# thawro/pytorch-human-pose

Measured on AMD Instinct MI355X. Metric: images/sec (fwd+decode) HigherHRNet-W32 512px, higher is better.
Workload: dtype bf16; 1 GPU; HigherHRNet-W32 inference bf16, batch 32 @ 512x512 per GPU (conv fwd on N(0,1) images + AE decode on constructed maps, 10 people/image, det_thr 0.05, tag_thr 0.5, adjust+refine); global_batch=32, parallelism=image-sharded replicas x1, no data-path collective

## Files before the change

### pytorch-human-pose_amd/csrc/engine.cpp

```cpp
#include "engine.h"

#include <cmath>
#include <cstdlib>
#include <cstring>

static thread_local std::string g_err;
LaunchProbe &hh_launch_probe()
{
    static thread_local LaunchProbe p;
    return p;
}
void hh_set_error(const std::string &msg) { g_err = msg; }
const char *hh_get_error() { return g_err.c_str(); }

PlanSwitches PlanSwitches::from_env()
{
    auto on = [](const char *name) { const char *v = getenv(name); return v && *v && strcmp(v, "0"); };
    auto is = [](const char *name, const char *val) { const char *v = getenv(name); return v && !strcmp(v, val); };
    PlanSwitches s;
    s.bb32_tile = is("HH_BB32", "tile");
    s.no_bb64 = on("HH_NO_BB64");
    s.no_bb_fp8 = on("HH_NO_BB_FP8");
    s.no_stem_fused = on("HH_NO_STEM_FUSED");
    s.no_junc_pair = on("HH_NO_JUNC_PAIR");
    s.full_join = on("HH_FULL_JOIN");
    s.no_fusion_merge = on("HH_NO_FUSION_MERGE");
    s.no_fused_upsum = on("HH_NO_FUSED_UPSUM");
    s.poison_ws = on("HH_POISON_WS");
    s.poison_lds = on("HH_POISON_LDS");
    s.no_head_fold = on("HH_NO_HEAD_FOLD");
    s.no_conv_db = on("HH_NO_CONV_DB");
    s.no_final_fuse = on("HH_NO_FINAL_FUSE");
    s.keep_waits = on("HH_KEEP_WAITS");
    s.event_system_fence = on("HH_EVENT_SYSTEM_FENCE");
    s.bb_tall = on("HH_NO_BB_TALL") ? 0 : is("HH_BB_TALL", "always") ? 2 : 1;
    if (const char *fc = getenv("HH_FAT_CUS")) { s.fat_cus = s.fat_cus64 = atoi(fc); if (const char *c2 = strchr(fc, ',')) s.fat_cus64 = atoi(c2 + 1); }
    if (const char *sk = getenv("HH_DEBUG_SKIP")) {
        static const struct { const char *name; unsigned bit; } cats[] = {{"s2big", SK_S2BIG}, {"s2", SK_S2}, {"upadd", SK_UPADD}, {"c1x1", SK_C1X1},
            {"c256", SK_C256}, {"c128", SK_C128}, {"junc", SK_JUNC}, {"bb32", SK_BB32}, {"bb64", SK_BB64}, {"stem", SK_STEM}, {"deconv", SK_DECONV},
            {"head", SK_HEAD}, {"trans0", SK_TRANS0}, {"upsum", SK_UPSUM}};
        std::string v = std::string(",") + sk + ",";
        for (const auto &c : cats)
            if (v.find(std::string(",") + c.name + ",") != std::string::npos) s.debug_skip |= c.bit;
    }
    s.fp8_trunk8 = is("HH_FP8_TRUNK", "e4m3");
    s.fp8_heads8 = is("HH_FP8_HEADS", "e4m3");
    return s;
}

static inline int round_up(int v, int m) { return (v + m - 1) / m * m; }

static inline bf16_raw f2bf(float f)
{
    uint32_t u;
    memcpy(&u, &f, 4);
    if ((u & 0x7fffffffu) > 0x7f800000u) return (bf16_raw)((u >> 16) | 0x40);
    u += 0x7fffu + ((u >> 16) & 1u);
    return (bf16_raw)(u >> 16);
}
static inline float bf2f(bf16_raw h)
{
    uint32_t u = (uint32_t)h << 16;
    float f;
    memcpy(&f, &u, 4);
    return f;
}

int hh_net::add_param(const std::string &name, std::vector<int64_t> shape, bool counter)
{
    ParamSlot p;
    p.name = name;
    p.shape = std::move(shape);
    p.counter = counter;
    param_index[name] = (int)params.size();
    params.push_back(std::move(p));
    return (int)params.size() - 1;
// ... 501 lines not shown
                for (int c8 = 0; c8 < C8; ++c8)
                    for (int ci_o = 0; ci_o < COUT_T; ++ci_o)
                        for (int j = 0; j < 8; ++j, ++o) {
                            const int co = cg * COUT_T + ci_o, ci = ch * KC + c8 * 8 + j;
                            if (co >= cout || ci >= cin) continue;
                            float v;
                            if (transposed) v = W[(((size_t)ci * cout + co) * 4 + ky) * 4 + kx];
                            else v = W[(((size_t)co * cin + ci) * ks + ky) * ks + kx];
                            packed[o] = f2bf(v * scale[co]);
                        }
            }
}

int hh_family_pick(int ks, int stride, int cin_pad, int coutp, int *KC, int *NT)
{
    if (ks == 3 && stride == 1) *KC = (cin_pad % 32 == 0) ? 32 : 16;
    else if (ks == 1) *KC = (cin_pad % 32 == 0) ? 32 : 16;
    else *KC = 16;
    *NT = (coutp % 64 == 0) ? 2 : 1;
    for (int i = 0; i < conv_num_configs(); ++i) {
        const ConvConfig &c = conv_config(i);
        if (c.KS == ks && c.S == stride && c.KC == *KC && c.NT == *NT && !c.DB) return 0;
    }
    return 1;
}

float hh_net::bn_fold(const std::string &bn, int co, const float *cb, float *shift) const
{
    const float g = param(bn + ".weight")[co], bta = param(bn + ".bias")[co];
    const float mu = param(bn + ".running_mean")[co], var = param(bn + ".running_var")[co];
    const float sc = g / std::sqrt(var + 1e-5f);
    *shift = cb ? bta + (*cb - mu) * sc : bta - mu * sc;
    return sc;
}

void hh_net::fold_layer(const ConvLayer &l, int coutp, std::vector<float> &scale, std::vector<float> &shift) const
{
    scale.assign(coutp, 0.f);
    shift.assign(coutp, 0.f);
    for (int co = 0; co < l.cout; ++co) {
        const float cb = l.bias.empty() ? 0.f : param(l.bias)[co];
        if (l.bn.empty()) { scale[co] = 1.f; shift[co] = cb; }
        else scale[co] = bn_fold(l.bn, co, &cb, &shift[co]);
    }
}

int hh_net::finalize()
{
    for (auto &p : params)
        if (!p.loaded && !p.counter) { hh_set_error("hh_finalize: parameter never loaded: " + p.name); return 1; }
    HH_CHECK_HIP(conv_init());
    HH_CHECK_HIP(bb_fused_init());
    HH_CHECK_HIP(stem_fused_init());
    HH_CHECK_HIP(bbpc_init());
    HH_CHECK_HIP(bb64_fused_init());
    HH_CHECK_HIP(junction_init());
    if (dtype == 2 && kind != 0) { hh_set_error("hh_finalize: the fp8 path covers HigherHRNet only"); return 1; }
    {
        int dev = 0;
        hipDeviceProp_t prop;
        HH_CHECK_HIP(hipGetDevice(&dev));
        HH_CHECK_HIP(hipGetDeviceProperties(&prop, dev));
        num_cus = prop.multiProcessorCount;
    }
    for (auto &l : layers) {
        if (l.stem) {
            const std::vector<float> &W = param(l.conv + ".weight");
            std::vector<bf16_raw> packed(64 * 32, 0);
            std::vector<float> shift(64);
            for (int co = 0; co < 64; ++co) {
                const float sc = bn_fold(l.bn, co, nullptr, &shift[co]);
                for (int t = 0; t < 27; ++t) {
                    const int kk = t / 16, hh = (t % 16) / 8, j = t % 8;
                    packed[((((co / 32) * 2 + kk) * 2 + hh) * 32 + co % 32) * 8 + j] = f2bf(W[(size_t)co * 27 + t] * sc);
                }
            }
            if (hh_upload(&l.d_w, packed.data(), packed.size() * 2) || hh_upload(&l.d_bias, shift.data(), 64 * 4)) return 1;
            continue;
        }
        if (dtype == 2 && !l.hi) continue;
        const int cin_pad0 = round_up(l.cin, 16), coutp = round_up(l.cout, 32);
        if (l.stem2) { l.KC = 64; l.NT = 2; }
        else if (hh_family_pick(l.ks, l.stride, cin_pad0, coutp, &l.KC, &l.NT)) {
            hh_set_error("no kernel family for conv " + l.conv);
            return 1;
        }
        l.db = !sw.no_conv_db && !l.stem2 && l.ks == 3 && l.stride == 1 && !l.transposed && l.mconv.empty() && l.cin >= 128 &&
               l.cin % 16 == 0 && coutp % 64 == 0;
        if (l.db) { l.KC = 16; l.NT = 2; }
        l.cin_pad = round_up(l.cin, l.KC);
        const int COUT_T = 32 * l.NT;
        l.ncg = coutp / COUT_T;
        if (!l.mconv.empty()) {
            std::vector<float> Wm((size_t)l.cout * l.cin * 9, 0.f), one(coutp, 1.f), shift(coutp, 0.f);
            int c0 = 0;
            for (size_t m = 0; m < l.mconv.size(); ++m) {
                if (l.mcin[m] % l.KC) { hh_set_error("merged fusion conv: input width not a multiple of the chunk size"); return 1; }
                const std::vector<float> &Wj = param(l.mconv[m] + ".weight");
                for (int co = 0; co < l.cout; ++co) {
                    float sh;
                    const float sc = bn_fold(l.mbn[m], co, nullptr, &sh);
                    shift[co] += sh;
                    for (int ci = 0; ci < l.mcin[m]; ++ci)
                        for (int t = 0; t < 9; ++t) Wm[((size_t)co * l.cin + c0 + ci) * 9 + t] = Wj[((size_t)co * l.mcin[m] + ci) * 9 + t] * sc;
                }
                c0 += l.mcin[m];
// ... 267 lines not shown
            }
            HH_CHECK_HIP(launch_avgpool(ti.ptr, ti.C, d_pool, B, (H >> ti.shift) * (W >> ti.shift), op.C, s));
            break;
        }
        case OP_LINEAR:
            HH_CHECK_HIP(launch_linear(d_pool, d_fc_w, d_fc_b, o1, B, 2048, num_classes, s));
            break;
        case OP_STEM: rc = enqueue_stem(op, images, B, H, W, s); break;
        case OP_UPADD: rc = dtype == 2 ? enqueue_fp8_upadd(op, B, H, W, s) : enqueue_upadd(op, B, H, W, s); break;
        case OP_UPSUM: rc = enqueue_upsum(op, B, H, W, s); break;
        case OP_JUNC: rc = enqueue_junc(op, B, H, W, s); break;
        case OP_BB: rc = dtype == 2 ? enqueue_fp8_bb(op, B, H, W, s) : enqueue_bb(op, B, H, W, o2, multi, s, &fin_done); break;
        case OP_QUANT: rc = enqueue_fp8_quant(op, B, H, W, s); break;
        case OP_CONV: rc = dtype == 2 && !op.hi ? enqueue_fp8_conv(op, B, H, W, o1, o2, s) : enqueue_conv(op, B, H, W, o1, o2, s); break;
        }
        if (rc) return 1;
    }
    if (multi)
        for (int l = 1; l < lc.open; ++l)
            if ((lc.dep(0, l) || sw.keep_waits) && lane_wait(0, l)) return 1;
    return 0;
}

int hh_net::prof_record(const Op &op, int cfg, const OpCost &c, unsigned long long **clk)
{
    if (prof_used == prof.size()) {
        ProfRecord r{};
        HH_CHECK_HIP(hipEventCreate(&r.e0));
        HH_CHECK_HIP(hipEventCreate(&r.e1));
        prof.push_back(r);
    }
    ProfRecord &r = prof[prof_used++];
    r.op = (int)(&op - ops.data());
    r.cfg = cfg;
    r.flops = c.flops;
    r.bytes = c.bytes;
    r.slot = clk && prof_used <= HH_PROF_SLOTS ? (int)prof_used - 1 : -1;
    if (r.slot >= 0 && prof_clk) *clk = d_clk + 4 * r.slot;
    hh_launch_probe() = LaunchProbe{r.e0, r.e1};
    return 0;
}

int hh_net::enqueue_stem(const Op &op, const float *images, int B, int H, int W, hipStream_t s)
{
    const ConvLayer &l = layers[op.layer];
    if (op.layer2 >= 0) {
        const ConvLayer &l2 = layers[op.layer2];
        StemFusedParams q{};
        q.images = images; q.w1 = l.d_w; q.b1 = l.d_bias; q.w2 = l2.d_w; q.b2 = l2.d_bias;
        q.out = tensors[op.out].ptr; q.out_cs = tensors[op.out].C;
        q.B = B; q.H = H; q.W = W;
        if (!stem_fused_supported(q)) { hh_set_error("hh_forward: the fused stem needs H, W multiples of 4 and images below 2 GB (HH_NO_STEM_FUSED=1)"); return 1; }
        if (prof_enabled && prof_record(op, HH_CFG_STEM_FUSED, op_cost(op, B, H, W), &q.clk)) return 1;
        HH_CHECK_HIP(stem_fused_launch(q, num_cus, s));
        return 0;
    }
    StemParams p{};
    p.images = images; p.w = l.d_w; p.bias = l.d_bias;
    p.out = tensors[op.out].ptr; p.out_cs = tensors[op.out].C;
    p.B = B; p.H = H; p.W = W;
    if (dtype == 2) {
        p.out_fp8 = (unsigned char *)tensors[op.out].ptr; p.out_inv_scale = 1.f / op.s_out;
        if (calibrating) p.absmax = d_amax + (&op - ops.data());
    }
    if (prof_enabled && prof_record(op, HH_CFG_STEM, op_cost(op, B, H, W), &p.clk)) return 1;
    HH_CHECK_HIP(stem_conv_launch(p, s));
    return 0;
}

int hh_net::enqueue_upadd(const Op &op, int B, int H, int W, hipStream_t s)
{
    UpAddParams p{};
    const TensorDesc &b = tensors[op.in], &o = tensors[op.out];
    p.base = b.ptr; p.base_cs = b.C; p.base_coff = 0;
    p.nup = op.nup;
    for (int j = 0; j < op.nup; ++j) {
        p.up[j] = tensors[op.up[j]].ptr; p.up_cs[j] = tensors[op.up[j]].C; p.up_shift[j] = op.up_shift[j];
    }
    p.out = o.ptr; p.out_cs = o.C; p.out_coff = 0;
    p.B = B; p.H = H >> b.shift; p.W = W >> b.shift; p.C = op.C; p.relu = op.relu;
    HH_CHECK_HIP(launch_upadd(p, s));
    return 0;
}

int hh_net::enqueue_upsum(const Op &op, int B, int H, int W, hipStream_t s)
{
    const TensorDesc &b0 = tensors[op.in], &o = tensors[op.out];
    FusionUpParams p{};
    p.x0 = b0.ptr; p.x0_cs = b0.C;
    p.nsrc = op.nup;
    for (int j = 0; j < op.nup; ++j) {
        const ConvLayer &l = layers[op.up_layer[j]];
        const TensorDesc &t = tensors[op.up[j]];
        if (t.shift != b0.shift + j + 1 || l.KC != 32 || l.NT != 1 || l.ncg != 1 || l.cin != (op.C << (j + 1))) {
            hh_set_error("plan: fusion output 0 does not fit fusion_up.hip (HH_NO_FUSED_UPSUM=1)");
            return 1;
        }
        p.src[j] = t.ptr; p.src_cs[j] = t.C; p.w[j] = l.d_w; p.bias[j] = l.d_bias;
    }
    p.out = o.ptr; p.out_cs = o.C;
    p.B = B; p.H = H >> b0.shift; p.W = W >> b0.shift;
    if (prof_enabled && prof_record(op, HH_CFG_FUSION_UP, op_cost(op, B, H, W), &p.clk)) return 1;
    HH_CHECK_HIP(fusion_up_launch(p, s));
    return 0;
}

int hh_net::enqueue_junc(const Op &op, int B, int H, int W, hipStream_t s)
// ... 20 lines not shown
int hh_net::enqueue_bb(const Op &op, int B, int H, int W, float *o2, bool multi, hipStream_t s, int *fin_done)
{
    const ConvLayer &l1 = layers[op.layer], &l2 = layers[op.layer2];
    const TensorDesc &ti = tensors[op.in], &to = tensors[op.out];
    BBParams p{};
    p.in = ti.ptr; p.in_cs = ti.C; p.out = to.ptr; p.out_cs = to.C;
    p.w1 = l1.d_w; p.w2 = l2.d_w; p.b1 = l1.d_bias; p.b2 = l2.d_bias;
    p.B = B; p.H = H >> ti.shift; p.W = W >> ti.shift;
    p.tall = sw.bb_tall;
    if (op.fin >= 0 && !sw.no_final_fuse && !sw.bb32_tile && !taps_enabled && o2 && !(sw.debug_skip & SK_HEAD)) {
        const ConvLayer &lf = layers[ops[op.fin].layer];
        p.fin_w = lf.d_wfin; p.fin_b = lf.d_bias; p.fin_out = o2; p.fin_K = lf.cout;
        if (lf.d_wfin && bbpc_final_supported(p)) *fin_done = op.fin;
        else { p.fin_w = nullptr; p.fin_b = nullptr; p.fin_out = nullptr; p.fin_K = 0; }
    }
    const int cfg = l1.cout == 64 ? HH_CFG_BB64_FUSED : HH_CFG_BB_FUSED;
    if (prof_enabled && prof_record(op, cfg, op_cost(op, B, H, W, p.fin_out != nullptr), &p.clk)) return 1;
    auto budget = [&](int want) { return !(multi && op.siblings) ? num_cus : want > 0 ? (want < num_cus ? want : num_cus) : (num_cus + 1) / 2; };
    const int fat = budget(sw.fat_cus), fat64 = budget(sw.fat_cus64);
    if (l1.cout == 64) HH_CHECK_HIP(bb64_fused_launch(p, fat64, s));
    else if (!sw.bb32_tile && bbpc_supported(p)) HH_CHECK_HIP(bbpc_launch(p, fat, s));
    else HH_CHECK_HIP(bb_fused_launch(p, num_cus, s));
    return 0;
}

int hh_net::enqueue_conv(const Op &op, int B, int H, int W, float *o1, float *o2, hipStream_t s)
{
    const ConvLayer &l = layers[op.layer];
    const TensorDesc &ti = tensors[op.in];
    ConvParams p{};
    hh_conv_geometry(p, l, op, B, H >> ti.shift, W >> ti.shift, o1, o2);
    p.in = dtype == 2 ? ti.ptr16 : ti.ptr; p.in_cs = ti.C; p.in_coff = op.in_coff;
    p.w = l.d_w; p.bias = l.d_bias;
    if (op.out >= 0) {
        const TensorDesc &to = tensors[op.out];
        p.out = dtype == 2 ? to.ptr16 : to.ptr; p.out_cs = to.C; p.out_coff = op.out_coff;
    }
    if (op.res >= 0) {
        const TensorDesc &tr = tensors[op.res];
        p.res = dtype == 2 ? tr.ptr16 : tr.ptr; p.res_cs = tr.C; p.res_coff = op.res_coff;
    }
    if (op.in2 >= 0) {
        const TensorDesc &t2 = tensors[op.in2];
        if (t2.C != ti.C || t2.shift != ti.shift || (op.in3 >= 0 && (tensors[op.in3].C != ti.C || tensors[op.in3].shift != ti.shift))) {
            hh_set_error("merged fusion conv: inputs differ in shape or pixel stride");
            return 1;
        }
        p.nch0 = l.mcin[0] / l.KC;
        p.nch1 = l.mcin[1] / l.KC;
        p.src_delta1 = t2.ptr - (ti.ptr + op.in_coff);
        if (op.in3 >= 0) p.src_delta2 = tensors[op.in3].ptr - (ti.ptr + op.in_coff);
    }
    p.cout_store = op.cout_store >= 0 ? op.cout_store : round_up(l.cout, 8);
    const int cfg = hh_pick_config(l.ks, l.stride, l.KC, l.NT, p.Wo, l.db);
    const ConvConfig &c = conv_config(cfg);
    p.tiles_x = (p.Wo + c.TW - 1) / c.TW;
    p.tiles_y = (p.Ho + c.th() - 1) / c.th();
    if (prof_enabled && prof_record(op, cfg, op_cost(op, B, H, W), &p.clk)) return 1;
    HH_CHECK_HIP(conv_launch(cfg, p, s));
    return 0;
}

int hh_net::forward(const float *images, int B, int H, int W, float *o1, float *o2, int use_graph, hipStream_t s)
{
    if (!finalized) { hh_set_error("hh_forward: call hh_finalize first"); return 1; }
    if (dtype == 2 && !calibrated) { hh_set_error("hh_forward: fp8 handle without activation scales, call hh_calibrate first"); return 1; }
    if (B > rB || H > rH || W > rW || !ws_ready || (taps_enabled && !taps.empty() && !taps[0].copy))
        if (reserve(B, H, W)) return 1;
    lastB = B; lastH = H; lastW = W;
    if (!use_graph || s == nullptr || taps_enabled || prof_enabled || sw.poison_lds || sw.debug_skip || multi_lane)
        return enqueue(images, B, H, W, o1, o2, s);
    for (auto &g : graphs)
        if (g.images == images && g.o1 == o1 && g.o2 == o2 && g.B == B && g.H == H && g.W == W) {
            HH_CHECK_HIP(hipGraphLaunch(g.exec, s));
            return 0;
        }
    hipGraph_t graph;
    HH_CHECK_HIP(hipStreamBeginCapture(s, hipStreamCaptureModeThreadLocal));
    const int rc = enqueue(images, B, H, W, o1, o2, s);
    hipError_t e = hipStreamEndCapture(s, &graph);
    if (rc) return rc;
    HH_CHECK_HIP(e);
    GraphEntry g{images, o1, o2, B, H, W, nullptr};
    HH_CHECK_HIP(hipGraphInstantiate(&g.exec, graph, nullptr, nullptr, 0));
    hipGraphDestroy(graph);
    if (graphs.size() >= 8) {
        HH_CHECK_HIP(hipStreamSynchronize(s));
        hipGraphExecDestroy(graphs.front().exec);
        graphs.erase(graphs.begin());
    }
    graphs.push_back(g);
    HH_CHECK_HIP(hipGraphLaunch(g.exec, s));
    return 0;
}

int hh_net::check_plan(std::string *why) const
{
    struct Stamp { int lane; int t; int op; };
    LaneClocks lc;
    auto before = [&](const Stamp &st, int lane) { return st.lane < 0 || lc.behind(lane, st.lane, st.t); };
    std::vector<Stamp> writer(tensors.size(), Stamp{-1, 0, -1});
    std::vector<std::vector<Stamp>> readers(tensors.size());
    for (size_t i = 0; i < ops.size(); ++i) {
        const Op &op = ops[i];
        if (op.kind == OP_JOIN) { lc.join(op.nlanes); continue; }
        if (op.kind == OP_DEP) { lc.dep(op.lane, op.dep_from); continue; }
// ... 170 lines not shown
```

### pytorch-human-pose_amd/csrc/engine.h

```cpp
#pragma once
#include <map>
#include <string>
#include <vector>

#include "kernels.h"

void hh_set_error(const std::string &msg);
void hh_pack_weights(const float *W, const float *scale, int ks, int cin, int cout, int KC, int COUT_T, bool transposed,
                     int py, int px, std::vector<unsigned short> &packed);
#define HH_CHECK_HIP(expr)                                                                             \
    do {                                                                                               \
        hipError_t _e = (expr);                                                                        \
        if (_e != hipSuccess) {                                                                        \
            hh_set_error(std::string(#expr) + ": " + hipGetErrorString(_e));                           \
            return 1;                                                                                  \
        }                                                                                              \
    } while (0)

struct ParamSlot {
    std::string name;
    std::vector<int64_t> shape;
    std::vector<float> data;
    bool loaded = false;
    bool counter = false;
// ... 41 lines not shown
    int layer4 = -1;
    int in2 = -1, out2 = -1;
    int in3 = -1;
    int in = -1, in_coff = 0;
    int out = -1, out_coff = 0;
    int res = -1, res_coff = 0;
    int relu = 0;
    int f32_out = 0;
    int cout_store = -1;
    int scatter = 0;
    int up[3] = {-1, -1, -1}, up_shift[3] = {0, 0, 0}, nup = 0;
    int up_layer[3] = {-1, -1, -1};
    int C = 0;
    int tap = -1;
    bool res8 = false;
    int fin = -1;
    bool siblings = false;
    bool hi = false;
    int lane = 0;
    int nlanes = 0;
    int dep_from = 0;
    float s_in = 1.f, s_in2 = 1.f, s_res = 1.f, s_out = 1.f, s_up[3] = {1.f, 1.f, 1.f};
    float s_mid = 1.f;
    int amax_slot = -1;
};

struct TapInfo {
    std::string name;
    int tensor, coff, C;
    bf16_raw *copy = nullptr;
    float scale = 1.f;
    bool is16 = false;
};

struct ProfRecord {
    int op, cfg;
    double flops, bytes;
    hipEvent_t e0, e1;
    int slot;
};

struct GraphEntry {
    const void *images;
    void *o1, *o2;
    int B, H, W;
    hipGraphExec_t exec;
};

struct PlanSwitches {
    bool bb32_tile = false;
    bool no_bb64 = false;
    bool no_bb_fp8 = false;
    bool no_stem_fused = false;
    bool no_junc_pair = false;
    bool full_join = false;
    bool no_fusion_merge = false;
    bool no_fused_upsum = false;
    bool poison_ws = false;
    int fat_cus = 0, fat_cus64 = 0;
    bool event_system_fence = false;
    bool keep_waits = false;
    bool no_final_fuse = false;
    int bb_tall = 1;
    bool no_conv_db = false;
    bool no_head_fold = false;
    bool poison_lds = false;
    unsigned debug_skip = 0;
    bool fp8_trunk8 = false;
    bool fp8_heads8 = false;
    static PlanSwitches from_env();
};

enum SkipCat { SK_S2BIG = 1, SK_S2 = 2, SK_UPADD = 4, SK_C1X1 = 8, SK_C256 = 16, SK_C128 = 32, SK_JUNC = 64, SK_BB32 = 128, SK_BB64 = 256,
               SK_STEM = 512, SK_DECONV = 1024, SK_HEAD = 2048, SK_TRANS0 = 4096, SK_UPSUM = 8192 };
inline unsigned hh_skip_cats(const Op &op, const std::vector<ConvLayer> &layers, const std::vector<TensorDesc> &tensors)
{
    switch (op.kind) {
    case OP_UPADD: return SK_UPADD;
    case OP_UPSUM: return SK_UPSUM;
    case OP_JUNC: return SK_JUNC;
    case OP_STEM: return SK_STEM;
    case OP_BB: return layers[op.layer].cout == 32 ? SK_BB32 : layers[op.layer].cout == 64 ? SK_BB64 : 0;
    case OP_CONV: break;
    default: return 0;
    }
    const ConvLayer &l = layers[op.layer];
    if (l.transposed) return SK_DECONV;
    if (op.f32_out) return SK_HEAD;
    if (l.stride == 2) return SK_S2 | (l.cin >= 128 ? SK_S2BIG : 0) | (l.cin == 256 && l.mconv.empty() && tensors[op.in].shift == 2 ? SK_TRANS0 : 0);
    if (l.ks == 1) return SK_C1X1;
    if (l.cin == 256 && l.cout == 256) return SK_C256;
    if (l.cin == 128 && l.cout == 128) return SK_C128;
    if (l.cin == 256 && tensors[op.in].shift == 2) return SK_TRANS0;
    return 0;
}

struct OpCost { double flops = 0, bytes = 0; };

struct hh_net {
    int K, C, dtype;
    int kind = 0;
    int num_classes = 0;
    float *d_pool = nullptr, *d_fc_w = nullptr, *d_fc_b = nullptr;
    int pool_cap = 0;
    std::vector<ParamSlot> params;
    std::map<std::string, int> param_index;
// ... 97 lines not shown
```

### pytorch-human-pose_amd/csrc/kernels.h

```cpp
#pragma once
#include <hip/hip_runtime.h>
#include <stdint.h>

#include <hip/hip_ext.h>

typedef uint16_t bf16_raw;

struct LaunchProbe { hipEvent_t start = nullptr, stop = nullptr; };
LaunchProbe &hh_launch_probe();
#define HH_LAUNCH(kernel, grid, block, lds, stream, ...)                                                            \
    do {                                                                                                            \
        LaunchProbe &lp_ = hh_launch_probe();                                                                       \
        if (lp_.start) {                                                                                            \
            hipExtLaunchKernelGGL(kernel, grid, block, lds, stream, lp_.start, lp_.stop, 0, __VA_ARGS__);           \
            lp_ = LaunchProbe{};                                                                                    \
        } else {                                                                                                    \
            hipLaunchKernelGGL(kernel, grid, block, lds, stream, __VA_ARGS__);                                      \
        }                                                                                                           \
    } while (0)

struct ConvParams {
    const bf16_raw *in;
    int in_cs, in_coff;
    int Hin, Win;
    const bf16_raw *w;
    const float *bias;
    const bf16_raw *res;
    int res_cs, res_coff;
    bf16_raw *out;
    int out_cs, out_coff;
    float *out_f32;
    int Hob, Wob;
    int osy, ooy, osx, oox;
    int Ho, Wo;
    int cin;
    int cout_real, cout_store;
    int relu;
    int pad_y, pad_x;
    int B, tiles_x, tiles_y, ncg;
    int nphase;
    size_t phase_stride;
    unsigned long long *stamps;
    unsigned long long *clk;
    int nch0, nch1;
    ptrdiff_t src_delta1, src_delta2;
};

struct ConvConfig {
    int KS, S, KC, NT, WC, PT, TW;
    int DB;
    int cout_t() const { return 32 * NT * WC; }
    int th() const { return (4 / WC) * PT * (32 / TW); }
    size_t lds_bytes() const {
        int PH = (th() - 1) * S + KS, PW = (TW - 1) * S + KS;
        size_t patch = ((size_t)PH * PW * (KC * 2 + 16) + 15) & ~(size_t)15;
        const size_t buf = patch + (size_t)KS * KS * KC * cout_t() * 2;
        return DB ? 2 * (buf + 256 * 16) : buf;
    }
};

int conv_num_configs();
const ConvConfig &conv_config(int i);
hipError_t conv_launch(int cfg_index, const ConvParams &p, hipStream_t stream);
hipError_t conv_init();

struct Fp8ConvParams {
    const unsigned char *in;
    int in_cs, in_coff;
    int Hin, Win;
    const unsigned char *w;
    const float *mult;
    const float *bias;
    const unsigned char *res;
    int res_cs, res_coff;
    float res_scale;
    const bf16_raw *res16;
    int res16_cs, res16_coff;
    unsigned char *out;
    int out_cs, out_coff;
    float out_inv_scale;
    bf16_raw *out16;
    int out16_cs, out16_coff;
    float *out_f32;
    int Hob, Wob;
    int osy, ooy, osx, oox;
    int Ho, Wo;
    int cin;
    int cout_real, cout_store;
    int relu;
    int pad_y, pad_x;
    int B, tiles_x, tiles_y, ncg;
    int nphase;
    size_t phase_stride;
    unsigned *absmax;
};
struct Fp8ConvConfig {
    int KS, S, KC, NT, PT, TW;
    static constexpr int pixel_stride(int kc) { return ((kc / 16 + 1) | 1) * 16; }
    int cout_t() const { return 32 * NT; }
    int th() const { return 4 * PT * (32 / TW); }
    int nstep() const { return (KS * KS * (KC / 16) + 3) / 4; }
    size_t lds_bytes() const {
        const int PH = (th() - 1) * S + KS, PW = (TW - 1) * S + KS;
        const size_t patch = ((size_t)PH * PW * pixel_stride(KC) + 15) & ~(size_t)15;
        return patch + (size_t)nstep() * 4 * cout_t() * 16;
    }
};
int conv_fp8_num_configs();
const Fp8ConvConfig &conv_fp8_config(int i);
hipError_t conv_fp8_launch(int cfg_index, const Fp8ConvParams &p, hipStream_t stream);
hipError_t conv_fp8_init();

struct Fp8BBParams {
    const unsigned char *in; int in_cs;
    unsigned char *out; int out_cs;
    const unsigned char *w1, *w2;
// ... 56 lines not shown
hipError_t bb_fused_init();
hipError_t bb_fused_launch(BBParams p, int num_cus, hipStream_t s);
hipError_t bbpc_init();
bool bbpc_supported(const BBParams &p);
bool bbpc_final_supported(const BBParams &p);
hipError_t bbpc_launch(BBParams p, int num_cus, hipStream_t s);
#define HH_CFG_BB64_FUSED 103
hipError_t bb64_fused_init();
hipError_t bb64_fused_launch(BBParams p, int num_cus, hipStream_t s);

struct JuncParams {
    const bf16_raw *t2; int t2_cs;
    const bf16_raw *res; int res_cs;
    const bf16_raw *x; int x_cs;
    const bf16_raw *t2a; int t2a_cs;
    const bf16_raw *w3a; const float *b3a;
    const bf16_raw *w3, *wd, *w1;
    const float *b3, *bd, *b1;
    bf16_raw *y; int y_cs;
    bf16_raw *t1; int t1_cs;
    int npix;
    unsigned long long *clk;
};
#define HH_CFG_JUNCTION 101
hipError_t junction_init();
hipError_t junction_launch(const JuncParams &p, int num_cus, hipStream_t s);

struct StemParams {
    const float *images;
    const bf16_raw *w;
    const float *bias;
    bf16_raw *out; int out_cs;
    int B, H, W;
    unsigned long long *clk;
    unsigned char *out_fp8;
    float out_inv_scale;
    unsigned *absmax;
};
#define HH_CFG_STEM 102
hipError_t stem_conv_launch(const StemParams &p, hipStream_t s);
struct StemFusedParams {
    const float *images;
    const bf16_raw *w1;
    const float *b1;
    const bf16_raw *w2;
    const float *b2;
    bf16_raw *out; int out_cs;
    int B, H, W;
    unsigned long long *clk;
};
#define HH_CFG_STEM_FUSED 106
hipError_t stem_fused_init();
bool stem_fused_supported(const StemFusedParams &p);
hipError_t stem_fused_launch(const StemFusedParams &p, int num_cus, hipStream_t s);


struct UpAddParams {
    const bf16_raw *base; int base_cs, base_coff;
    const bf16_raw *up[3]; int up_cs[3]; int up_shift[3]; int nup;
    bf16_raw *out; int out_cs, out_coff;
    int B, H, W, C, relu;
};
hipError_t launch_upadd(const UpAddParams &p, hipStream_t s);
struct FusionUpParams {
    const bf16_raw *x0; int x0_cs;
    const bf16_raw *src[3];
    int src_cs[3];
    const bf16_raw *w[3];
    const float *bias[3];
    int nsrc;
    bf16_raw *out; int out_cs;
    int B, H, W;
    int tiles_x, tiles_y;
    unsigned long long *clk;
};
#define HH_CFG_FUSION_UP 107
bool fusion_up_supported(int C, int nsrc);
hipError_t fusion_up_launch(FusionUpParams p, hipStream_t s);
hipError_t launch_upadd_backward(const bf16_raw *dy, const bf16_raw *out, int relu, int B, int H, int W, int C, bf16_raw *g, bf16_raw *const *dup,
                                 const int *up_shift, int nup, hipStream_t s);
struct UpAddFp8Params {
    const unsigned char *base; int base_cs; float base_scale;
    const unsigned char *up[3]; int up_cs[3]; int up_shift[3]; float up_scale[3]; int nup;
    const bf16_raw *base16; int base16_cs;
    const bf16_raw *up16[3]; int up16_cs[3];
    unsigned char *out; int out_cs;
    float out_inv_scale;
    bf16_raw *out16; int out16_cs;
    int B, H, W, C, relu;
    unsigned *absmax;
};
hipError_t launch_upadd_fp8(const UpAddFp8Params &p, hipStream_t s);
hipError_t launch_quant_fp8(const bf16_raw *in, int in_cs, unsigned char *out, int out_cs, size_t npix, int C, float inv_scale, unsigned *absmax,
                            hipStream_t s);

hipError_t launch_lds_poison(int num_cus, hipStream_t s);
hipError_t launch_avgpool(const bf16_raw *in, int in_cs, float *out, int B, int HW, int C, hipStream_t s);
hipError_t launch_linear(const float *x, const float *w, const float *bias, float *y, int B, int K, int N, hipStream_t s);

struct HHImageDesc {
    long long offset;
    int h, w;
    double inv[6];
};
hipError_t launch_preprocess_batch(const unsigned char *base, const HHImageDesc *descs, int n, float *out, int H, int W,
                                   const float mean[3], const float stdv[3], hipStream_t s);
hipError_t launch_warp_affine_u8(const unsigned char *img, int h, int w, const double inv[6], unsigned char *out, int H, int W, hipStream_t s);
// ... 68 lines not shown
```

### pytorch-human-pose_amd/csrc/stem_fused.hip

```cpp
#include "mfma_dev.h"

namespace {
constexpr int T2H = 2, T2W = 32;
constexpr int MR = 2 * T2H + 1, MC = 2 * T2W + 1;
constexpr int MPIX = MR * MC, NQ = (MPIX + 31) / 32;
constexpr int PRW = 4 * T2H + 3, PCW = 4 * T2W + 3;
constexpr int PLANE = PRW * PCW, NVAL = 3 * PLANE;
constexpr int NLD = (NVAL + 255) / 256;
constexpr int PS2 = 144, HALF = (MC + 1) / 2;
constexpr int MID_BYTES = MR * 2 * HALF * PS2;
constexpr int PATCH_BYTES = ((NVAL + 1) * 2 + 15) / 16 * 16;
constexpr int OFF_PATCH = MID_BYTES, OFF_BIAS = OFF_PATCH + PATCH_BYTES, LDS_BYTES = OFF_BIAS + 2 * 64 * 4;
constexpr int RD = 3, NFB = RD + 1;
}

__global__ __launch_bounds__(256, 1) void stem_fused_kernel(const StemFusedParams p)
{
    extern __shared__ __attribute__((aligned(16))) char smem[];
    unsigned short *patch = reinterpret_cast<unsigned short *>(smem + OFF_PATCH);
    const int tid = threadIdx.x;
#ifndef HH_NO_CLK
    if (p.clk && tid == 0) atomicMin(p.clk, wall_clock64());
#endif
    const int lds0 = (int)(size_t)(__attribute__((address_space(3))) char *)smem;
// ... 104 lines not shown
            const int my = mc / MC, mx = mc - my * MC;
            const int gy = 2 * g.oy0 - 1 + my, gx = 2 * g.ox0 - 1 + mx;
            const bool inside = ((unsigned)gy < (unsigned)H1) & ((unsigned)gx < (unsigned)W1);
            char *dst = smem + ((my * 2 + (mx & 1)) * HALF + (mx >> 1)) * PS2 + h * 16;
#pragma unroll
            for (int ct = 0; ct < 2; ++ct) {
                f32x16 acc = bias1[ct];
#pragma unroll
                for (int kk = 0; kk < 2; ++kk)
                    acc = __builtin_amdgcn_mfma_f32_32x32x16_bf16(__builtin_bit_cast(bf16x8, a1[ct][kk]), __builtin_bit_cast(bf16x8, bf[qi][kk]), acc, 0, 0, 0);
                u32x4 o[2];
                pack_rows16(acc, o);
                if (m < MPIX) {
                    *reinterpret_cast<u32x4 *>(dst + ct * 64) = inside ? o[0] : u32x4{0u, 0u, 0u, 0u};
                    *reinterpret_cast<u32x4 *>(dst + ct * 64 + 32) = inside ? o[1] : u32x4{0u, 0u, 0u, 0u};
                }
            }
        }
        __syncthreads();

        patch_write();

        {
            f32x16 acc = bias_acc(64 + ct2 * 32);
            const int ma = lds0 + (row2 * 4 * HALF + r) * PS2 + h * 16;
            u32x4 fb[NFB];
            auto ldb = [&](auto sc, int buf) {
                constexpr int s = decltype(sc)::value, tap = s >> 2, kk = s & 3, ky = tap / 3, kx = tap % 3;
                fb[buf] = lds_read_async<((ky * 2 + (kx & 1)) * HALF + (kx >> 1)) * PS2 + kk * 32>(ma);
            };
            static_for<RD>([&](auto sc) { ldb(sc, decltype(sc)::value); });
            static_for<36>([&](auto sc) {
                constexpr int s = decltype(sc)::value;
                if constexpr (s + RD < 36) ldb(std::integral_constant<int, s + RD>{}, (s + RD) % NFB);
                lds_wait<(35 - s < RD ? 35 - s : RD)>(fb[s % NFB]);
                acc = __builtin_amdgcn_mfma_f32_32x32x16_bf16(__builtin_bit_cast(bf16x8, w2r[s]), __builtin_bit_cast(bf16x8, fb[s % NFB]), acc, 0, 0, 0);
            });
            u32x4 o[2];
            pack_rows16(acc, o);
            const int oy = g.oy0 + row2, ox = g.ox0 + r;
            const bool ok = (oy < H2) & (ox < W2);
            const auto rs_out = __builtin_amdgcn_make_buffer_rsrc(p.out + (size_t)g.b * out_elems, 0, (int)(out_elems * 2), 0x00020000);
            const unsigned voff = ok ? (unsigned)(((oy * W2 + ox) * p.out_cs + ct2 * 32 + 8 * h) * 2) : OOB;
            __builtin_amdgcn_raw_buffer_store_b128(o[0], rs_out, (int)voff, 0, 0);
            __builtin_amdgcn_raw_buffer_store_b128(o[1], rs_out, (int)voff, 32, 0);
        }
        __syncthreads();
    }
#ifndef HH_NO_CLK
    if (p.clk && tid == 0) atomicMax(p.clk + 1, wall_clock64());
#endif
}

hipError_t stem_fused_init()
{
    return hipFuncSetAttribute(reinterpret_cast<const void *>(stem_fused_kernel), hipFuncAttributeMaxDynamicSharedMemorySize, LDS_BYTES);
}

bool stem_fused_supported(const StemFusedParams &p)
{
    return p.H % 4 == 0 && p.W % 4 == 0 && (size_t)3 * p.H * p.W * 4 < 0x7fffffffull && (size_t)(p.H / 4) * (p.W / 4) * p.out_cs * 2 < 0x7fffffffull;
}

hipError_t stem_fused_launch(const StemFusedParams &p, int num_cus, hipStream_t s)
{
    const int H2 = p.H >> 2, W2 = p.W >> 2;
    const int ntiles = p.B * ((H2 + T2H - 1) / T2H) * ((W2 + T2W - 1) / T2W);
    const int grid = ntiles < num_cus ? ntiles : num_cus;
    HH_LAUNCH(stem_fused_kernel, dim3(grid), dim3(256), LDS_BYTES, s, p);
    return hipGetLastError();
}
```

Measured before the change: 6902 images/sec.

## Add warp-specialized producer/consumer stem and persistent 64-channel 3x3 conv kernel

```diff
diff --git a/pytorch-human-pose_amd/csrc/conv64_ws.hip b/pytorch-human-pose_amd/csrc/conv64_ws.hip
--- /dev/null
+++ b/pytorch-human-pose_amd/csrc/conv64_ws.hip
@@ -0,0 +1,156 @@
+#include "mfma_dev.h"
+
+namespace {
+constexpr int WS_TH = 8, WS_TW = 32, WS_PH = WS_TH + 2, WS_PW = WS_TW + 2;
+constexpr int WS_PS = 64 * 2 + 16;
+constexpr int WS_PATCH = WS_PH * WS_PW * WS_PS;
+constexpr int WS_UNITS = WS_PH * WS_PW * 8;
+constexpr int WS_NPL = (WS_UNITS + 511) / 512;
+constexpr int WS_OFF_BIAS = 2 * WS_PATCH, WS_LDS = WS_OFF_BIAS + 64 * 4;
+constexpr int WS_NS = 48, WS_RD = 3, WS_NFB = WS_RD + 1;
+static_assert(WS_PATCH % 16 == 0 && WS_LDS <= 160 * 1024, "16-byte aligned buffers inside the CU's LDS");
+}
+
+__global__ __launch_bounds__(512, 1) void conv64_ws_kernel(const ConvParams p)
+{
+    extern __shared__ __attribute__((aligned(16))) char smem[];
+    const int tid = threadIdx.x;
+#ifndef HH_NO_CLK
+    if (p.clk && tid == 0) atomicMin(p.clk, wall_clock64());
+#endif
+    const int lds0 = (int)(size_t)(__attribute__((address_space(3))) char *)smem;
+    const int wave = __builtin_amdgcn_readfirstlane(tid >> 6), lane = tid & 63, r = lane & 31, h = lane >> 5;
+    const int rp = wave >> 1, ct = wave & 1;
+
+    u32x4 wr[36];
+    {
+        const auto rs_w = __builtin_amdgcn_make_buffer_rsrc(const_cast<bf16_raw *>(p.w), 0, 2 * 9 * 4 * 64 * 16, 0x00020000);
+        static_for<36>([&](auto fc) {
+            constexpr int f = decltype(fc)::value, c = f / 3, ky = f % 3, chunk = c / 6, kx = (c / 2) % 3, kk = c & 1;
+            wr[f] = __builtin_bit_cast(u32x4, __builtin_amdgcn_raw_buffer_load_b128(rs_w, ((((chunk * 9 + ky * 3 + kx) * 4 + kk * 2 + h) * 64) + ct * 32 + r) * 16, 0, 0));
+        });
+    }
+    if (tid < 64) reinterpret_cast<float *>(smem + WS_OFF_BIAS)[tid] = p.bias[tid];
+    const short fl = p.relu ? (short)0 : (short)-32768;
+    const i16x2 floor = {fl, fl};
+
+    const int tiles_img = p.tiles_x * p.tiles_y, ntiles = p.B * tiles_img;
+    const int nloc = (ntiles - (int)blockIdx.x + (int)gridDim.x - 1) / (int)gridDim.x;
+    struct Geom { int b, oy0, ox0; };
+    auto geom = [&](int k) {
+        int i = (int)blockIdx.x + k * (int)gridDim.x;
+        i = i < ntiles ? i : ntiles - 1;
+        const int t = ((ntiles & 7) == 0 && (gridDim.x & 7) == 0) ? (i & 7) * (ntiles >> 3) + (i >> 3) : i;
+        const int tt = t % tiles_img;
+        return Geom{t / tiles_img, (tt / p.tiles_x) * WS_TH, (tt % p.tiles_x) * WS_TW};
+    };
+
+    u32x4 preg[WS_NPL];
+    unsigned pmask = 0;
+    const bf16_raw *in_b = p.in + p.in_coff;
+    int iy0 = 0, ix0 = 0;
+    auto stage_tile = [&](int k) {
+        const Geom g = geom(k);
+        in_b = p.in + (size_t)g.b * p.Hin * p.Win * p.in_cs + p.in_coff;
+        iy0 = g.oy0 - 1; ix0 = g.ox0 - 1;
+    };
+    auto load_unit = [&](auto jc) {
+        constexpr int j = decltype(jc)::value;
+        const int u = tid + 512 * j, pix = u >> 3, part = u & 7;
+        const int iy = iy0 + pix / WS_PW, ix = ix0 + pix % WS_PW;
+        const bool ok = u < WS_UNITS && iy >= 0 && iy < p.Hin && ix >= 0 && ix < p.Win;
+        preg[j] = *reinterpret_cast<const u32x4 *>(ok ? in_b + ((size_t)iy * p.Win + ix) * p.in_cs + part * 8 : in_b);
+        pmask = (pmask & ~(1u << j)) | (ok ? (1u << j) : 0u);
+    };
+    auto write_unit = [&](auto jc, int buf) {
+        constexpr int j = decltype(jc)::value;
+        const int u = tid + 512 * j;
+        if (u < WS_UNITS)
+            *reinterpret_cast<u32x4 *>(smem + buf * WS_PATCH + (u >> 3) * WS_PS + (u & 7) * 16) = (pmask >> j) & 1u ? preg[j] : u32x4{0u, 0u, 0u, 0u};
+    };
+
+    stage_tile(0);
+    static_for<WS_NPL>([&](auto jc) { load_unit(jc); });
+    static_for<WS_NPL>([&](auto jc) { write_unit(jc, 0); });
+    stage_tile(1);
+    static_for<WS_NPL>([&](auto jc) { load_unit(jc); });
+    lds_barrier();
+
+    for (int k = 0; k < nloc; ++k) {
+        const Geom g = geom(k);
+        stage_tile(k + 2);
+        f32x16 acc[2];
+#pragma unroll
+        for (int q = 0; q < 4; ++q) {
+            const float4 bv = *reinterpret_cast<const float4 *>(smem + WS_OFF_BIAS + (ct * 32 + 8 * q + 4 * h) * 4);
+            acc[0][4 * q + 0] = bv.x + 0.f; acc[0][4 * q + 1] = bv.y + 0.f; acc[0][4 * q + 2] = bv.z + 0.f; acc[0][4 * q + 3] = bv.w + 0.f;
+        }
+        acc[1] = acc[0];
+        const int ma = lds0 + (k & 1) * WS_PATCH + ((2 * rp) * WS_PW + r) * WS_PS + h * 16;
+        u32x4 fb[WS_NFB];
+        auto ldb = [&](auto sc, int buf) {
+            constexpr int s = decltype(sc)::value, c = s >> 2, i = s & 3, chunk = c / 6, kx = (c / 2) % 3, kk = c & 1;
+            fb[buf] = lds_read_async<(i * WS_PW + kx) * WS_PS + chunk * 64 + kk * 32>(ma);
+        };
+        static_for<WS_RD>([&](auto sc) { ldb(sc, decltype(sc)::value); });
+        static_for<WS_NS>([&](auto sc) {
+            constexpr int s = decltype(sc)::value, c = s >> 2, i = s & 3;
+            if constexpr (s + WS_RD < WS_NS) ldb(std::integral_constant<int, s + WS_RD>{}, (s + WS_RD) % WS_NFB);
+            if constexpr (s % 8 == 4 && s / 8 < WS_NPL) {
+                write_unit(std::integral_constant<int, s / 8>{}, (k + 1) & 1);
+                load_unit(std::integral_constant<int, s / 8>{});
+            }
+            lds_wait<(WS_NS - 1 - s < WS_RD ? WS_NS - 1 - s : WS_RD)>(fb[s % WS_NFB]);
+            static_for<3>([&](auto kyc) {
+                constexpr int ky = decltype(kyc)::value, pt = i - ky;
+                if constexpr (pt >= 0 && pt < 2)
+                    acc[pt] = __builtin_amdgcn_mfma_f32_32x32x16_bf16(__builtin_bit_cast(bf16x8, wr[c * 3 + ky]), __builtin_bit_cast(bf16x8, fb[s % WS_NFB]), acc[pt], 0, 0, 0);
+            });
+        });
+        const int ox = g.ox0 + r;
+#pragma unroll
+        for (int pt = 0; pt < 2; ++pt) {
+            const int oy = g.oy0 + 2 * rp + pt;
+            const bool valid = oy < p.Ho && ox < p.Wo;
+            const size_t pix = ((size_t)g.b * p.Ho + oy) * p.Wo + ox;
+#pragma unroll
+            for (int m = 0; m < 2; ++m) {
+                const unsigned x0 = pack_bf16x2(acc[pt][8 * m + 0], acc[pt][8 * m + 1], floor);
+                const unsigned x1 = pack_bf16x2(acc[pt][8 * m + 2], acc[pt][8 * m + 3], floor);
+                const unsigned y0 = pack_bf16x2(acc[pt][8 * m + 4], acc[pt][8 * m + 5], floor);
+                const unsigned y1 = pack_bf16x2(acc[pt][8 * m + 6], acc[pt][8 * m + 7], floor);
+                auto s0 = __builtin_amdgcn_permlane32_swap(x0, y0, false, false);
+                auto s1 = __builtin_amdgcn_permlane32_swap(x1, y1, false, false);
+                if (valid)
+                    *reinterpret_cast<u32x4 *>(p.out + pix * p.out_cs + p.out_coff + ct * 32 + 16 * m + 8 * h) = u32x4{s0[0], s1[0], s0[1], s1[1]};
+            }
+        }
+        lds_barrier();
+    }
+#ifndef HH_NO_CLK
+    if (p.clk && tid == 0) atomicMax(p.clk + 1, wall_clock64());
+#endif
+}
+
+hipError_t conv64_ws_init()
+{
+    return hipFuncSetAttribute(reinterpret_cast<const void *>(conv64_ws_kernel), hipFuncAttributeMaxDynamicSharedMemorySize, WS_LDS);
+}
+
+bool conv64_ws_supported(const ConvParams &p)
+{
+    return p.cin == 64 && p.cout_real == 64 && p.cout_store == 64 && p.ncg == 1 && p.nphase <= 1 && p.nch0 == 0 && !p.res && !p.out_f32 && p.out &&
+           p.osy == 1 && p.osx == 1 && p.ooy == 0 && p.oox == 0 && p.pad_y == 1 && p.pad_x == 1 && p.Ho == p.Hin && p.Wo == p.Win &&
+           p.Hob == p.Ho && p.Wob == p.Wo && p.in_cs % 8 == 0 && p.in_coff % 8 == 0 && p.out_cs % 8 == 0 && p.out_coff % 8 == 0;
+}
+
+hipError_t conv64_ws_launch(ConvParams p, int num_cus, int max_wgs, hipStream_t s)
+{
+    p.tiles_x = (p.Wo + WS_TW - 1) / WS_TW;
+    p.tiles_y = (p.Ho + WS_TH - 1) / WS_TH;
+    const int ntiles = p.B * p.tiles_x * p.tiles_y;
+    int grid = ntiles < num_cus ? ntiles : num_cus;
+    if (max_wgs > 0 && grid > max_wgs) grid = max_wgs;
+    HH_LAUNCH(conv64_ws_kernel, dim3(grid), dim3(512), WS_LDS, s, p);
+    return hipGetLastError();
+}
diff --git a/pytorch-human-pose_amd/csrc/engine.cpp b/pytorch-human-pose_amd/csrc/engine.cpp
--- a/pytorch-human-pose_amd/csrc/engine.cpp
+++ b/pytorch-human-pose_amd/csrc/engine.cpp
@@ -22,6 +22,9 @@
     s.no_bb64 = on("HH_NO_BB64");
     s.no_bb_fp8 = on("HH_NO_BB_FP8");
     s.no_stem_fused = on("HH_NO_STEM_FUSED");
+    s.no_stem_pc = on("HH_NO_STEM_PC");
+    s.no_conv2_ws = on("HH_NO_CONV2_WS");
+    if (const char *pw = getenv("HH_PREFIX_WGS")) s.prefix_wgs = atoi(pw);
     s.no_junc_pair = on("HH_NO_JUNC_PAIR");
     s.full_join = on("HH_FULL_JOIN");
     s.no_fusion_merge = on("HH_NO_FUSION_MERGE");
@@ -629,6 +632,7 @@
     HH_CHECK_HIP(conv_init());
     HH_CHECK_HIP(bb_fused_init());
     HH_CHECK_HIP(stem_fused_init());
+    HH_CHECK_HIP(conv64_ws_init());
     HH_CHECK_HIP(bbpc_init());
     HH_CHECK_HIP(bb64_fused_init());
     HH_CHECK_HIP(junction_init());
@@ -1002,7 +1006,7 @@
         q.B = B; q.H = H; q.W = W;
         if (!stem_fused_supported(q)) { hh_set_error("hh_forward: the fused stem needs H, W multiples of 4 and images below 2 GB (HH_NO_STEM_FUSED=1)"); return 1; }
         if (prof_enabled && prof_record(op, HH_CFG_STEM_FUSED, op_cost(op, B, H, W), &q.clk)) return 1;
-        HH_CHECK_HIP(stem_fused_launch(q, num_cus, s));
+        HH_CHECK_HIP(stem_fused_launch(q, num_cus, !sw.no_stem_pc, sw.prefix_wgs, s));
         return 0;
     }
     StemParams p{};
@@ -1129,6 +1133,12 @@
         if (op.in3 >= 0) p.src_delta2 = tensors[op.in3].ptr - (ti.ptr + op.in_coff);
     }
     p.cout_store = op.cout_store >= 0 ? op.cout_store : round_up(l.cout, 8);
+    if (dtype != 2 && !sw.no_conv2_ws && l.ks == 3 && l.stride == 1 && !l.transposed && l.cin == 64 && l.cout == 64 && l.KC == 32 && l.NT == 2 &&
+        !l.db && op.in2 < 0 && conv64_ws_supported(p)) {
+        if (prof_enabled && prof_record(op, HH_CFG_CONV64_WS, op_cost(op, B, H, W), &p.clk)) return 1;
+        HH_CHECK_HIP(conv64_ws_launch(p, num_cus, sw.prefix_wgs, s));
+        return 0;
+    }
     const int cfg = hh_pick_config(l.ks, l.stride, l.KC, l.NT, p.Wo, l.db);
     const ConvConfig &c = conv_config(cfg);
     p.tiles_x = (p.Wo + c.TW - 1) / c.TW;
diff --git a/pytorch-human-pose_amd/csrc/engine.h b/pytorch-human-pose_amd/csrc/engine.h
--- a/pytorch-human-pose_amd/csrc/engine.h
+++ b/pytorch-human-pose_amd/csrc/engine.h
@@ -117,6 +117,9 @@
     bool no_bb64 = false;
     bool no_bb_fp8 = false;
     bool no_stem_fused = false;
+    bool no_stem_pc = false;
+    bool no_conv2_ws = false;
+    int prefix_wgs = 0;
     bool no_junc_pair = false;
     bool full_join = false;
     bool no_fusion_merge = false;
diff --git a/pytorch-human-pose_amd/csrc/kernels.h b/pytorch-human-pose_amd/csrc/kernels.h
--- a/pytorch-human-pose_amd/csrc/kernels.h
+++ b/pytorch-human-pose_amd/csrc/kernels.h
@@ -62,6 +62,10 @@
 int conv_num_configs();
 const ConvConfig &conv_config(int i);
 hipError_t conv_launch(int cfg_index, const ConvParams &p, hipStream_t stream);
+#define HH_CFG_CONV64_WS 108
+hipError_t conv64_ws_init();
+bool conv64_ws_supported(const ConvParams &p);
+hipError_t conv64_ws_launch(ConvParams p, int num_cus, int max_wgs, hipStream_t s);
 hipError_t conv_init();
 
 struct Fp8ConvParams {
@@ -224,7 +228,7 @@
 #define HH_CFG_STEM_FUSED 106
 hipError_t stem_fused_init();
 bool stem_fused_supported(const StemFusedParams &p);
-hipError_t stem_fused_launch(const StemFusedParams &p, int num_cus, hipStream_t s);
+hipError_t stem_fused_launch(const StemFusedParams &p, int num_cus, bool pc, int max_wgs, hipStream_t s);
 
 
 struct UpAddParams {
diff --git a/pytorch-human-pose_amd/csrc/stem_fused.hip b/pytorch-human-pose_amd/csrc/stem_fused.hip
--- a/pytorch-human-pose_amd/csrc/stem_fused.hip
+++ b/pytorch-human-pose_amd/csrc/stem_fused.hip
@@ -180,9 +180,187 @@
 #endif
 }
 
+namespace {
+constexpr int PC_OFF_PATCH = 2 * MID_BYTES, PC_OFF_BIAS = PC_OFF_PATCH + 2 * PATCH_BYTES, PC_LDS_BYTES = PC_OFF_BIAS + 2 * 64 * 4;
+static_assert(PC_LDS_BYTES <= 160 * 1024 && MID_BYTES % 16 == 0 && PATCH_BYTES % 16 == 0, "LDS budget / 16-byte aligned buffers");
+}
+
+__global__ __launch_bounds__(512, 1) void stem_fused_pc_kernel(const StemFusedParams p)
+{
+    extern __shared__ __attribute__((aligned(16))) char smem[];
+    const int tid = threadIdx.x;
+#ifndef HH_NO_CLK
+    if (p.clk && tid == 0) atomicMin(p.clk, wall_clock64());
+#endif
+    const int lds0 = (int)(size_t)(__attribute__((address_space(3))) char *)smem;
+    const int wave = __builtin_amdgcn_readfirstlane(tid >> 6), lane = tid & 63, r = lane & 31, h = lane >> 5;
+    const int H1 = p.H >> 1, W1 = p.W >> 1, H2 = p.H >> 2, W2 = p.W >> 2;
+    const size_t img_elems = (size_t)3 * p.H * p.W, out_elems = (size_t)H2 * W2 * p.out_cs;
+    constexpr unsigned OOB = 0x80000000u;
+
+    if (tid < 64) {
+        reinterpret_cast<float *>(smem + PC_OFF_BIAS)[tid] = p.b1[tid];
+        reinterpret_cast<float *>(smem + PC_OFF_BIAS)[64 + tid] = p.b2[tid];
+    }
+    if (tid < 2) reinterpret_cast<unsigned short *>(smem + PC_OFF_PATCH + tid * PATCH_BYTES)[NVAL] = 0;
+    auto bias_acc = [&](int off) {
+        f32x16 b0;
+#pragma unroll
+        for (int q = 0; q < 4; ++q) {
+            const float4 bv = *reinterpret_cast<const float4 *>(smem + PC_OFF_BIAS + (off + 8 * q + 4 * h) * 4);
+            b0[4 * q + 0] = bv.x; b0[4 * q + 1] = bv.y; b0[4 * q + 2] = bv.z; b0[4 * q + 3] = bv.w;
+        }
+        return b0;
+    };
+
+    const int tiles_x = (W2 + T2W - 1) / T2W, tiles_y = (H2 + T2H - 1) / T2H, ntiles = p.B * tiles_x * tiles_y;
+    const int nloc = (ntiles - (int)blockIdx.x + (int)gridDim.x - 1) / (int)gridDim.x;
+    struct Geom { int b, oy0, ox0; };
+    auto geom = [&](int k) {
+        const int i = (int)blockIdx.x + k * (int)gridDim.x;
+        const int t = ((ntiles & 7) == 0 && (gridDim.x & 7) == 0) ? (i & 7) * (ntiles >> 3) + (i >> 3) : i;
+        const int tx = t % tiles_x, ty = (t / tiles_x) % tiles_y;
+        return Geom{t / (tiles_x * tiles_y), ty * T2H, tx * T2W};
+    };
+
+    if (wave < 4) {
+        u32x4 a1[2][2];
+#pragma unroll
+        for (int ct = 0; ct < 2; ++ct)
+#pragma unroll
+            for (int kk = 0; kk < 2; ++kk) a1[ct][kk] = reinterpret_cast<const u32x4 *>(p.w1)[((ct * 2 + kk) * 2 + h) * 32 + r];
+        int off[2][8];
+#pragma unroll
+        for (int kk = 0; kk < 2; ++kk)
+#pragma unroll
+            for (int j = 0; j < 8; ++j) {
+                const int t = kk * 16 + 8 * h + j;
+                off[kk][j] = t < 27 ? (t / 9) * PLANE + ((t % 9) / 3) * PCW + (t % 3) : -1;
+            }
+        for (int k = -1; k <= nloc; ++k) {
+            if (k >= 0 && k < nloc) {
+                const Geom g = geom(k);
+                const unsigned short *patch = reinterpret_cast<const unsigned short *>(smem + PC_OFF_PATCH + (k & 1) * PATCH_BYTES);
+                char *mid = smem + (k & 1) * MID_BYTES;
+                constexpr int NQW = (NQ + 3) / 4;
+                u32x4 bf[NQW][2];
+#pragma unroll
+                for (int qi = 0; qi < NQW; ++qi) {
+                    const int q = wave + 4 * qi;
+                    const int m = q * 32 + r, mc = m < MPIX ? m : MPIX - 1;
+                    const int my = mc / MC, mx = mc - my * MC;
+                    const int base = (2 * my) * PCW + 2 * mx;
+#pragma unroll
+                    for (int kk = 0; kk < 2; ++kk) {
+                        unsigned short v[8];
+#pragma unroll
+                        for (int j = 0; j < 8; ++j) v[j] = patch[off[kk][j] >= 0 ? base + off[kk][j] : NVAL];
+                        bf[qi][kk] = u32x4{(unsigned)v[0] | ((unsigned)v[1] << 16), (unsigned)v[2] | ((unsigned)v[3] << 16),
+                                           (unsigned)v[4] | ((unsigned)v[5] << 16), (unsigned)v[6] | ((unsigned)v[7] << 16)};
+                    }
+                }
+                const f32x16 bias1[2] = {bias_acc(0), bias_acc(32)};
+#pragma unroll
+                for (int qi = 0; qi < NQW; ++qi) {
+                    const int q = wave + 4 * qi;
+                    if (q >= NQ) break;
+                    const int m = q * 32 + r, mc = m < MPIX ? m : MPIX - 1;
+                    const int my = mc / MC, mx = mc - my * MC;
+                    const int gy = 2 * g.oy0 - 1 + my, gx = 2 * g.ox0 - 1 + mx;
+                    const bool inside = ((unsigned)gy < (unsigned)H1) & ((unsigned)gx < (unsigned)W1);
+                    char *dst = mid + ((my * 2 + (mx & 1)) * HALF + (mx >> 1)) * PS2 + h * 16;
+#pragma unroll
+                    for (int ct = 0; ct < 2; ++ct) {
+                        f32x16 acc = bias1[ct];
+#pragma unroll
+                        for (int kk = 0; kk < 2; ++kk)
+                            acc = __builtin_amdgcn_mfma_f32_32x32x16_bf16(__builtin_bit_cast(bf16x8, a1[ct][kk]), __builtin_bit_cast(bf16x8, bf[qi][kk]), acc, 0, 0, 0);
+                        u32x4 o[2];
+                        pack_rows16(acc, o);
+                        if (m < MPIX) {
+                            *reinterpret_cast<u32x4 *>(dst + ct * 64) = inside ? o[0] : u32x4{0u, 0u, 0u, 0u};
+                            *reinterpret_cast<u32x4 *>(dst + ct * 64 + 32) = inside ? o[1] : u32x4{0u, 0u, 0u, 0u};
+                        }
+                    }
+                }
+            }
+            lds_barrier();
+        }
+    } else {
+        const int ctid = tid - 256, row2 = (wave >> 1) & 1, ct2 = wave & 1;
+        u32x4 w2r[36];
+        {
+            const auto rs_w = __builtin_amdgcn_make_buffer_rsrc(const_cast<bf16_raw *>(p.w2), 0, 9 * 8 * 64 * 16, 0x00020000);
+            static_for<36>([&](auto fc) {
+                constexpr int f = decltype(fc)::value, tap = f >> 2, kk = f & 3;
+                w2r[f] = __builtin_bit_cast(u32x4, __builtin_amdgcn_raw_buffer_load_b128(rs_w, (((tap * 8 + kk * 2 + h) * 64) + ct2 * 32 + r) * 16, 0, 0));
+            });
+        }
+        float pv[NLD];
+        auto patch_load = [&](int k) {
+            const Geom g = geom(k);
+            const auto rs_img = __builtin_amdgcn_make_buffer_rsrc(const_cast<float *>(p.images + (size_t)g.b * img_elems), 0, (int)(img_elems * 4), 0x00020000);
+            const int iy0 = 4 * g.oy0 - 3, ix0 = 4 * g.ox0 - 3;
+#pragma unroll
+            for (int it = 0; it < NLD; ++it) {
+                const int i = ctid + 256 * it;
+                const int c = i / PLANE, rem = i - c * PLANE, py = rem / PCW, px = rem - py * PCW;
+                const int iy = iy0 + py, ix = ix0 + px;
+                const bool ok = (i < NVAL) & ((unsigned)iy < (unsigned)p.H) & ((unsigned)ix < (unsigned)p.W);
+                const unsigned voff = ok ? (unsigned)(((c * p.H + iy) * p.W + ix) * 4) : OOB;
+                pv[it] = __builtin_bit_cast(float, __builtin_amdgcn_raw_buffer_load_b32(rs_img, (int)voff, 0, 0));
+            }
+        };
+        auto patch_write = [&](int buf) {
+            unsigned short *patch = reinterpret_cast<unsigned short *>(smem + PC_OFF_PATCH + buf * PATCH_BYTES);
+#pragma unroll
+            for (int it = 0; it < NLD; ++it) {
+                const int i = ctid + 256 * it;
+                if (it + 1 < NLD || i < NVAL) patch[i] = __builtin_bit_cast(unsigned short, (__bf16)pv[it]);
+            }
+        };
+        patch_load(0);
+        for (int k = -2; k < nloc; ++k) {
+            if (k + 2 < nloc) patch_write(k & 1);
+            if (k + 3 < nloc) patch_load(k + 3);
+            if (k >= 0) {
+                const Geom g = geom(k);
+                f32x16 acc = bias_acc(64 + ct2 * 32);
+                const int ma = lds0 + (k & 1) * MID_BYTES + (row2 * 4 * HALF + r) * PS2 + h * 16;
+                u32x4 fb[NFB];
+                auto ldb = [&](auto sc, int buf) {
+                    constexpr int s = decltype(sc)::value, tap = s >> 2, kk = s & 3, ky = tap / 3, kx = tap % 3;
+                    fb[buf] = lds_read_async<((ky * 2 + (kx & 1)) * HALF + (kx >> 1)) * PS2 + kk * 32>(ma);
+                };
+                static_for<RD>([&](auto sc) { ldb(sc, decltype(sc)::value); });
+                static_for<36>([&](auto sc) {
+                    constexpr int s = decltype(sc)::value;
+                    if constexpr (s + RD < 36) ldb(std::integral_constant<int, s + RD>{}, (s + RD) % NFB);
+                    lds_wait<(35 - s < RD ? 35 - s : RD)>(fb[s % NFB]);
+                    acc = __builtin_amdgcn_mfma_f32_32x32x16_bf16(__builtin_bit_cast(bf16x8, w2r[s]), __builtin_bit_cast(bf16x8, fb[s % NFB]), acc, 0, 0, 0);
+                });
+                u32x4 o[2];
+                pack_rows16(acc, o);
+                const int oy = g.oy0 + row2, ox = g.ox0 + r;
+                const bool ok = (oy < H2) & (ox < W2);
+                const auto rs_out = __builtin_amdgcn_make_buffer_rsrc(p.out + (size_t)g.b * out_elems, 0, (int)(out_elems * 2), 0x00020000);
+                const unsigned voff = ok ? (unsigned)(((oy * W2 + ox) * p.out_cs + ct2 * 32 + 8 * h) * 2) : OOB;
+                __builtin_amdgcn_raw_buffer_store_b128(o[0], rs_out, (int)voff, 0, 0);
+                __builtin_amdgcn_raw_buffer_store_b128(o[1], rs_out, (int)voff, 32, 0);
+            }
+            lds_barrier();
+        }
+    }
+#ifndef HH_NO_CLK
+    if (p.clk && tid == 256) atomicMax(p.clk + 1, wall_clock64());
+#endif
+}
+
 hipError_t stem_fused_init()
 {
-    return hipFuncSetAttribute(reinterpret_cast<const void *>(stem_fused_kernel), hipFuncAttributeMaxDynamicSharedMemorySize, LDS_BYTES);
+    hipError_t e = hipFuncSetAttribute(reinterpret_cast<const void *>(stem_fused_kernel), hipFuncAttributeMaxDynamicSharedMemorySize, LDS_BYTES);
+    if (e != hipSuccess) return e;
+    return hipFuncSetAttribute(reinterpret_cast<const void *>(stem_fused_pc_kernel), hipFuncAttributeMaxDynamicSharedMemorySize, PC_LDS_BYTES);
 }
 
 bool stem_fused_supported(const StemFusedParams &p)
@@ -190,11 +368,16 @@
     return p.H % 4 == 0 && p.W % 4 == 0 && (size_t)3 * p.H * p.W * 4 < 0x7fffffffull && (size_t)(p.H / 4) * (p.W / 4) * p.out_cs * 2 < 0x7fffffffull;
 }
 
-hipError_t stem_fused_launch(const StemFusedParams &p, int num_cus, hipStream_t s)
+hipError_t stem_fused_launch(const StemFusedParams &p, int num_cus, bool pc, int max_wgs, hipStream_t s)
 {
     const int H2 = p.H >> 2, W2 = p.W >> 2;
     const int ntiles = p.B * ((H2 + T2H - 1) / T2H) * ((W2 + T2W - 1) / T2W);
-    const int grid = ntiles < num_cus ? ntiles : num_cus;
-    HH_LAUNCH(stem_fused_kernel, dim3(grid), dim3(256), LDS_BYTES, s, p);
+    int grid = ntiles < num_cus ? ntiles : num_cus;
+    if (max_wgs > 0 && grid > max_wgs) grid = max_wgs;
+    if (pc) {
+        HH_LAUNCH(stem_fused_pc_kernel, dim3(grid), dim3(512), PC_LDS_BYTES, s, p);
+    } else {
+        HH_LAUNCH(stem_fused_kernel, dim3(grid), dim3(256), LDS_BYTES, s, p);
+    }
     return hipGetLastError();
 }
```

Result: no change. 6956 images/sec, median of 6 (+0.8%).
